# ramosian-glider/syzkaller

Hardware: AMD Instinct MI355X
Metric: coverage PCs triaged/sec vs corpus signal (+ % HBM roofline), 1/2/4/8 MI355X (higher is better)
Workload: dtype u32

## Files before the change

### syzkaller_amd/csrc/sg_bucket.hip

```cpp
#include "sg_part.h"

namespace sg {

#ifndef SG_BTHREADS
#define SG_BTHREADS 512
#endif
constexpr int kBThreads = SG_BTHREADS;
constexpr int kBWaves = kBThreads == 512 ? 6 : 8;
constexpr int kBU = 4;
constexpr uint32_t kHash = 8192;
constexpr uint32_t kMaxProbe = 31;
constexpr uint32_t kEmpty = 0xFFFFFFFFu;

struct BucketArgs {
  const uint32_t* in;
  const uint4* bdesc;
  const uint32_t* gbnd;
  uint32_t NG;
  uint32_t* mwords;
  const uint32_t* owords;
  uint32_t* nwords;
  uint8_t* rec_new;
  uint32_t* spill;
  uint32_t* nspill;
  uint32_t* ticket;
  const uint32_t* blist_b;
  const uint4* blist_q;
  const uint32_t* nlist;
  uint32_t win, win_shift;
  const uint32_t* fsum;
  uint64_t* dbg;
  uint2* pairs;
  unsigned long long* npairs;
  uint32_t rec_base;
  uint32_t nshards;
  unsigned long long* shard_cnt;
  uint32_t update;
  unsigned long long* gcur;
  const uint64_t* goff;
};

__device__ __forceinline__ uint32_t shard_of(uint32_t s, uint32_t nshards) {
  s ^= s >> 16;
  s *= 0x85EBCA6Bu;
  s ^= s >> 13;
  s *= 0xC2B2AE35u;
  s ^= s >> 16;
  return (uint32_t)(((uint64_t)s * nshards) >> 32);
}

constexpr uint32_t kMaxShards = 64;

template <int kPer>
__device__ __forceinline__ void emit_pairs(const BucketArgs& a, const uint32_t (&sig)[kPer], const uint32_t (&rec)[kPer],
                                           uint32_t* shcnt) {
  constexpr uint32_t kNone = 0xFFFFFFFFu;
  __shared__ uint32_t ewc[16];
  __shared__ unsigned long long ebase;
  const int lane = threadIdx.x & 63, w = threadIdx.x >> 6, nw = blockDim.x >> 6;
  uint32_t c = 0;
#pragma unroll
  for (int k = 0; k < kPer; k++) c += rec[k] != kNone ? 1u : 0u;
  uint32_t incl = c;
#pragma unroll
  for (int o = 1; o < 64; o <<= 1) {
    const uint32_t y = __shfl_up(incl, o);
    if (lane >= o) incl += y;
  }
  if (lane == 63) ewc[w] = incl;
  __syncthreads();
  if (threadIdx.x == 0) {
    uint32_t acc = 0;
    for (int i = 0; i < nw; i++) {
      const uint32_t v = ewc[i];
      ewc[i] = acc;
      acc += v;
    }
    ebase = acc ? atomicAdd(a.npairs, (unsigned long long)acc) : 0ull;
  }
  __syncthreads();
  uint64_t pos = ebase + ewc[w] + incl - c;
#pragma unroll
  for (int k = 0; k < kPer; k++)
    if (rec[k] != kNone) {
      a.pairs[pos++] = make_uint2(sig[k], a.rec_base + rec[k]);
      if (a.shard_cnt) atomicAdd(&shcnt[shard_of(sig[k], a.nshards)], 1u);
    }
  __syncthreads();
}

template <int kPer>
__device__ __forceinline__ void emit_grouped(const BucketArgs& a, const uint32_t (&sig)[kPer], const uint32_t (&rec)[kPer],
                                             uint32_t* lcnt, unsigned long long* lbase) {
  constexpr uint32_t kNone = 0xFFFFFFFFu;
#pragma unroll
  for (int k = 0; k < kPer; k++)
    if (rec[k] != kNone) atomicAdd(&lcnt[rec[k] >> kGroupBits], 1u);
  __syncthreads();
  for (uint32_t g = threadIdx.x; g < a.NG; g += blockDim.x) {
    const uint32_t c = lcnt[g];
    lbase[g] = c ? a.goff[(uint64_t)g << kGroupBits] + atomicAdd(&a.gcur[g], (unsigned long long)c) : 0ull;
    lcnt[g] = 0;
  }
  __syncthreads();
#pragma unroll
  for (int k = 0; k < kPer; k++)
    if (rec[k] != kNone) {
      const uint32_t g = rec[k] >> kGroupBits;
      a.pairs[lbase[g] + atomicAdd(&lcnt[g], 1u)] = make_uint2(sig[k], rec[k]);
    }
  __syncthreads();
  for (uint32_t g = threadIdx.x; g < a.NG; g += blockDim.x) lcnt[g] = 0;
  __syncthreads();
// ... 57 lines not shown
  for (int j = 0; j < kWPT; j++) {
    P.msw[j] = m[j];
    P.nsw[j] = nw[j];
  }
  const uint32_t* gr = a.gbnd + (uint64_t)b * a.NG;
#pragma unroll
  for (int j = 0; j < (int)kGroupWords; j++) {
    const uint32_t i = j * kBThreads + threadIdx.x;
    P.gw[j] = i < a.NG ? gr[i] : 0u;
  }
}

__device__ __forceinline__ uint32_t list_bucket(const BucketArgs& a, uint32_t t, uint32_t l0, uint32_t nl, uint4* q) {
  if (t >= nl) return kNumBuckets;
  *q = a.blist_q[l0 + t];
  return a.blist_b[l0 + t];
}

__device__ __forceinline__ bool fs_full(const uint32_t* fs, uint32_t rec) {
  return (fs[rec >> (kFsBits + 5)] >> ((rec >> kFsBits) & 31u)) & 1u;
}

__global__ __launch_bounds__(256) void k_flag_summary(const uint8_t* __restrict__ rec_new, uint32_t nrec,
                                                      uint32_t* __restrict__ sum, uint32_t* __restrict__ nfull) {
  const uint32_t blk = blockIdx.x * 4 + (threadIdx.x >> 6), lane = threadIdx.x & 63;
  if (blk >= (nrec + kFsRecs - 1) >> kFsBits) return;
  bool full = true;
#pragma unroll
  for (int j = 0; j < 4; j++) {
    const uint32_t i = blk * kFsRecs + j * 1024 + lane * 16;
    if (i + 16 <= nrec && ((uintptr_t)(rec_new + i) & 15) == 0) {
      const uint4 v = *reinterpret_cast<const uint4*>(rec_new + i);
      for (uint32_t w : {v.x, v.y, v.z, v.w}) full &= ((w - 0x01010101u) & ~w & 0x80808080u) == 0;
    } else {
      for (uint32_t k = i; k < i + 16 && k < nrec; k++) full &= rec_new[k] != 0;
    }
  }
  if (__all(full) && lane == 0) {
    atomicOr(&sum[blk >> 5], 1u << (blk & 31));
    atomicAdd(nfull, 1u);
  }
}

__device__ __forceinline__ uint4 uni(uint4 v) { return make_uint4(uni(v.x), uni(v.y), uni(v.z), uni(v.w)); }

constexpr uint32_t kMapMul = 0x6F4Bu;
constexpr uint32_t inv16(uint32_t c) {
  uint32_t x = c;
  for (int i = 0; i < 4; i++) x = (x * (2u - c * x)) & 0xFFFFu;
  return x;
}
constexpr uint32_t kMapInv = inv16(kMapMul);
static_assert(((kMapMul * kMapInv) & 0xFFFFu) == 1u, "kMapInv");
static_assert(kHash == 8192 && kMaxProbe <= 31, "13-bit slots, 5-bit displacements");
static_assert((uint64_t)kMaxGroups << kGroupBits <= (1u << 24), "records fit 24 bits");
constexpr uint32_t kRecMask = 0xFFFFFFu;

__device__ __forceinline__ uint32_t map_signal(uint32_t slot, uint32_t v) {
  const uint32_t home = (slot - ((v >> 24) & 31u)) & (kHash - 1);
  return (((home << 3) | (v >> 29)) * kMapInv) & 0xFFFFu;
}

__device__ __forceinline__ bool map_insert(uint32_t* ht, uint32_t sl, uint32_t rec, uint32_t disp0 = 0) {
  const uint32_t y = (sl * kMapMul) & 0xFFFFu;
  const uint32_t home = y >> 3, tag = y & 7u;
  for (uint32_t disp = disp0; disp < kMaxProbe; disp++) {
    const uint32_t mine = (tag << 29) | (disp << 24) | rec;
    uint32_t* slot = &ht[(home + disp) & (kHash - 1)];
    const uint32_t old = atomicCAS(slot, kEmpty, mine);
    if (old == kEmpty) return true;
    if ((old >> 24) == (mine >> 24)) {
      if ((old & kRecMask) > rec) atomicMin(slot, mine);
      return true;
    }
  }
  return false;
}

__device__ __forceinline__ uint32_t take_ticket(uint32_t* p) { return atomicAdd(p, 1u); }

template <bool kDbg, int kEmit, bool kSkip = false>
__global__ __launch_bounds__(kBThreads) __attribute__((amdgpu_waves_per_eu(kBWaves))) void k_bucket(BucketArgs a) {
  static_assert(!kSkip || kEmit == 0, "the summary guards flag stores");
  __shared__ uint32_t fsum[kSkip ? kFsWords : 1];
  __shared__ uint32_t mslice[kBucketWords];
  __shared__ uint32_t nbits[kBucketWords];
  __shared__ uint32_t ht[kHash];
  __shared__ alignas(16) uint32_t gb[kMaxGroups];
  __shared__ uint32_t sh_fail;
  __shared__ uint32_t sh_b[2];
  __shared__ uint4 sh_q[2];
  __shared__ uint32_t shcnt[kEmit == 1 ? kMaxShards : 1];
  __shared__ uint32_t lcnt[kEmit == 2 ? kMaxGroups : 1];
  __shared__ unsigned long long lbase[kEmit == 2 ? kMaxGroups : 1];
  const int tid = threadIdx.x;
  if (kEmit == 1)
    for (uint32_t i = tid; i < kMaxShards; i += kBThreads) shcnt[i] = 0;
  if (kEmit == 2)
    for (uint32_t i = tid; i < kMaxGroups; i += kBThreads) lcnt[i] = 0;
  const uint32_t NG = a.NG;
  constexpr uint32_t kRound = kBThreads * kBU;
  const uint64_t t_start = kDbg ? wall_clock64() : 0;
  uint64_t n_buckets = 0, n_rounds = 0;
  uint64_t ph[7] = {0, 0, 0, 0, 0, 0, 0};
  uint64_t tk = kDbg ? clock64() : 0;
  for (uint32_t i = tid; i < kHash; i += kBThreads) ht[i] = kEmpty;
  for (uint32_t i = tid; i < kBucketWords; i += kBThreads) nbits[i] = 0;
  if (tid == 0) sh_fail = 0;
  if (kSkip)
    for (uint32_t i = tid; i < kFsWords; i += kBThreads) fsum[i] = a.fsum[i];
  uint32_t nl = *a.nlist, l0 = 0;
  if (a.win) {
    const uint32_t na = nl >> a.win_shift;
    l0 = a.win == 2 ? na : 0;
    nl = a.win == 2 ? nl - na : na;
  }
  uint32_t pend_t = 0;
  if (tid == 0) {
    uint4 q0 = make_uint4(0, 0, 0, 0), q1 = make_uint4(0, 0, 0, 0);
    sh_b[0] = list_bucket(a, blockIdx.x, l0, nl, &q0);
    sh_q[0] = q0;
    sh_b[1] = list_bucket(a, gridDim.x + blockIdx.x, l0, nl, &q1);
    sh_q[1] = q1;
    pend_t = take_ticket(a.ticket);
  }
  __syncthreads();
  uint32_t b = uni(sh_b[0]), b1 = uni(sh_b[1]);
  uint4 q = uni(sh_q[0]), q1 = uni(sh_q[1]);
  if (b >= kNumBuckets) {
    if (kDbg && tid == 0) {
      for (int j = 0; j < 8; j++) a.dbg[8 * blockIdx.x + j] = 0;
      a.dbg[8 * blockIdx.x] = t_start;
      a.dbg[8 * blockIdx.x + 1] = wall_clock64();
    }
    return;
  }
  uint32_t x[kBU], y[kBU];
  BucketPre P;
  bucket_round_load(a, q.x & ~3u, q.y, x);
  bucket_pre_load(a, b, P);
  while (b < kNumBuckets) {
    const uint32_t lo = q.x, hi = q.y;
    __syncthreads();
    {
      wvec mv;
#pragma unroll
      for (int j = 0; j < kWPT; j++) mv[j] = P.msw[j];
      reinterpret_cast<wvec*>(mslice)[tid] = mv;
    }
    uint32_t ns[kWPT];
#pragma unroll
    for (int j = 0; j < kWPT; j++) ns[j] = P.nsw[j];
#pragma unroll
    for (int j = 0; j < (int)kGroupWords; j++) {
      const uint32_t i = j * kBThreads + tid;
      if (i < kMaxGroups) gb[i] = i < NG ? P.gw[j] : kEmpty;
    }
    uint32_t pend_b = kNumBuckets;
    uint4 pend_q = make_uint4(0, 0, 0, 0);
    if (tid == 0) {
      pend_b = list_bucket(a, 2 * gridDim.x + pend_t, l0, nl, &pend_q);
      pend_t = take_ticket(a.ticket);
      sh_fail = 0;
    }
    __syncthreads();
    const uint32_t gbl = NG <= 64 ? gb[threadIdx.x & 63] : kEmpty;
// ... 217 lines not shown
        for (int j = 0; j < kWPT; j++)
          if (nb[j]) {
            a.mwords[w0 + j] = mw[j] | nb[j];
            if (a.nwords) a.nwords[w0 + j] = ns[j] | nb[j];
          }
      } else if (a.nwords) {
        const wvec nb = reinterpret_cast<const wvec*>(nbits)[tid];
        uint32_t* ng = a.nwords + bucket_word(b, kWPT * tid);
#pragma unroll
        for (int j = 0; j < kWPT; j++)
          if (nb[j]) ng[j] = ns[j] | nb[j];
      }
      reinterpret_cast<wvec*>(nbits)[tid] = wvec{};
    } else {
      constexpr int kOwn = kHash / kBThreads;
      {
#pragma unroll
        for (int k = 0; k < kOwn; k++) {
          const uint32_t i = k * kBThreads + tid;
          const uint32_t v = ht[i];
          ht[i] = kEmpty;
          if (v != kEmpty) {
            const uint32_t sl = map_signal(i, v);
            atomicOr(&nbits[sl >> 5], 1u << (sl & 31));
            if (!kSkip || !fs_full(fsum, v & kRecMask)) a.rec_new[v & kRecMask] = 1;
          }
        }
        __syncthreads();
      }
      {
        const uint64_t w0 = bucket_word(b, kWPT * tid);
        uint32_t* mg = a.mwords + w0;
        uint32_t* ng = a.nwords ? a.nwords + w0 : nullptr;
        const wvec nb = reinterpret_cast<const wvec*>(nbits)[tid];
        uint32_t any = 0;
#pragma unroll
        for (int j = 0; j < kWPT; j++) any |= nb[j];
        if (any) {
          const wvec mw = reinterpret_cast<const wvec*>(mslice)[tid];
#pragma unroll
          for (int j = 0; j < kWPT; j++)
            if (nb[j]) {
              mg[j] = mw[j] | nb[j];
              if (ng) ng[j] = ns[j] | nb[j];
            }
          reinterpret_cast<wvec*>(nbits)[tid] = wvec{};
        }
      }
    }
    if (kDbg) {
      const uint64_t t = clock64();
      ph[3] += t - tk;
      tk = t;
    }
    __syncthreads();
    if (kDbg) {
      const uint64_t t = clock64();
      ph[6] += t - tk;
      tk = t;
    }
    b = b1;
    q = q1;
    b1 = uni(sh_b[0]);
    q1 = uni(sh_q[0]);
#pragma unroll
    for (int u = 0; u < kBU; u++) x[u] = y[u];
  }
  if (kEmit == 1) {
    __syncthreads();
    flush_shard_counts(a, shcnt);
  }
  if (kDbg && tid == 0) {
    a.dbg[8 * blockIdx.x] = t_start;
    a.dbg[8 * blockIdx.x + 1] = wall_clock64();
    a.dbg[8 * blockIdx.x + 2] = n_buckets;
    a.dbg[8 * blockIdx.x + 3] = n_rounds;
    for (int j = 0; j < 4; j++) a.dbg[8 * blockIdx.x + 4 + j] = ph[j];
    a.dbg[8 * gridDim.x + 3 * blockIdx.x] = ph[4];
    a.dbg[8 * gridDim.x + 3 * blockIdx.x + 1] = ph[5];
    a.dbg[8 * gridDim.x + 3 * blockIdx.x + 2] = ph[6];
  }
}

constexpr int kDThreads = 1024;
template <bool kEmit>
__global__ __launch_bounds__(kDThreads) void k_bucket_direct(BucketArgs a) {
  constexpr uint32_t kQ = 8192, kNQ = 65536 / kQ, kQW = kQ / 32;
  __shared__ uint32_t owner[kQ];
  __shared__ uint32_t mpart[kQW];
  __shared__ uint32_t nbits[kQW];
  __shared__ uint32_t gb[kMaxGroups];
  __shared__ uint32_t shcnt[kEmit ? kMaxShards : 1];
  __shared__ uint32_t lcnt[kEmit ? kMaxGroups : 1];
  __shared__ unsigned long long lbase[kEmit ? kMaxGroups : 1];
  __shared__ uint32_t fsum[kEmit ? 1 : kFsWords];
  const int tid = threadIdx.x;
  const uint32_t nsp = *a.nspill, NG = a.NG;
  if (!kEmit)
    for (uint32_t i = tid; i < kFsWords; i += kDThreads) fsum[i] = a.fsum ? a.fsum[i] : 0u;
  if (kEmit) {
    for (uint32_t i = tid; i < kMaxShards; i += kDThreads) shcnt[i] = 0;
    for (uint32_t i = tid; i < kMaxGroups; i += kDThreads) lcnt[i] = 0;
    __syncthreads();
  }
  for (uint32_t job = blockIdx.x; job < nsp * kNQ; job += gridDim.x) {
    const uint32_t b = a.spill[job / kNQ], qq = job % kNQ;
    const uint4 q = a.bdesc[b];
    for (uint32_t i = tid; i < kQW; i += kDThreads) {
      const uint64_t w = bucket_word(b, qq * kQW + i);
      mpart[i] = a.mwords[w] | (a.owords ? a.owords[w] : 0u);
      nbits[i] = 0;
    }
    for (uint32_t i = tid; i < NG; i += kDThreads) gb[i] = a.gbnd[(uint64_t)b * NG + i];
    for (uint32_t i = tid; i < kQ; i += kDThreads) owner[i] = kEmpty;
    __syncthreads();
    for (uint32_t i = q.x + tid; i < q.y; i += kDThreads) {
      const uint32_t x = a.in[i];
      const uint32_t sl = x >> 16, sq = sl % kQ;
      if (sl / kQ != qq || ((mpart[sq >> 5] >> (sq & 31)) & 1u)) continue;
      atomicMin(&owner[sq], entry_record(group_of(gb, NG, i), x));
      atomicOr(&nbits[sq >> 5], 1u << (sq & 31));
    }
    __syncthreads();
    if (kEmit) {
      constexpr int kPer = kQ / kDThreads;
      uint32_t sig[kPer], rec[kPer];
#pragma unroll
      for (int k = 0; k < kPer; k++) {
        const uint32_t i = k * kDThreads + tid;
        sig[k] = part_sig((b << 16) | (qq * kQ + i));
        rec[k] = owner[i];
      }
      if (a.gcur)
        emit_grouped(a, sig, rec, lcnt, lbase);
      else
        emit_pairs(a, sig, rec, shcnt);
      for (uint32_t i = tid; i < kQW; i += kDThreads) {
        const uint32_t nb = nbits[i];
        if (!nb) continue;
        const uint64_t w = bucket_word(b, qq * kQW + i);
        if (a.update) a.mwords[w] = mpart[i] | nb;
        if (a.nwords) a.nwords[w] |= nb;
      }
    } else {
      for (uint32_t i = tid; i < kQ; i += kDThreads)
        if (owner[i] != kEmpty && !fs_full(fsum, owner[i])) a.rec_new[owner[i]] = 1;
      for (uint32_t i = tid; i < kQW; i += kDThreads) {
        const uint32_t nb = nbits[i];
        if (nb) {
          const uint64_t w = bucket_word(b, qq * kQW + i);
          a.mwords[w] = mpart[i] | nb;
          if (a.nwords) a.nwords[w] |= nb;
        }
      }
    }
    __syncthreads();
  }
  if (kEmit) flush_shard_counts(a, shcnt);
}

uint32_t persistent_grid(sg_ctx* ctx, const void* kernel, int threads) {
  static std::mutex mu;
  static std::map<std::pair<int, const void*>, uint32_t> cache;
  std::lock_guard<std::mutex> lock(mu);
  const auto key = std::make_pair(ctx->device, kernel);
  auto it = cache.find(key);
// ... 4 lines not shown
  if (hipDeviceGetAttribute(&cus, hipDeviceAttributeMultiprocessorCount, ctx->device) != hipSuccess || cus < 1)
    cus = 256;
  const uint32_t grid = (uint32_t)(per_cu * cus);
  cache[key] = grid;
  return grid;
}

constexpr double kFsQueued = 0.9997;
static bool fs_split(sg_ctx* ctx) {
  const int64_t o = ctx->opt[kOptFlagSkip];
  if (o >= 0) return o != 0;
  m0f_poll(ctx);
  return ctx->m0f_queued >= kFsQueued;
}

int buckets_one(sg_ctx* ctx, const BucketPlan& bp, uint32_t* mwords, uint32_t* nwords, uint8_t* d_rec_new,
                const EmitArgs* emit, const uint32_t* owords) {
  const uint64_t nrec = bp.nrec;
  const uint32_t* gcount = bp.at<uint32_t>(ctx, kCB) + bp.ng;
  uint4* bdesc = bp.at<uint4>(ctx, kBD);
  uint32_t* nspill = bp.at<uint32_t>(ctx, kSP);
  const bool dbg = ctx->debug_part;
  BucketArgs ba{};
  ba.in = bp.at<uint32_t>(ctx, kV2);
  ba.bdesc = bdesc;
  ba.gbnd = bp.at<uint32_t>(ctx, kGB);
  ba.NG = (uint32_t)bp.NG;
  ba.mwords = mwords;
  ba.owords = owords;
  ba.nwords = nwords;
  ba.rec_new = d_rec_new;
  ba.nspill = nspill;
  ba.spill = nspill + 1;
  ba.ticket = bp.at<uint32_t>(ctx, kTK);
  if (emit) {
    ba.pairs = emit->pairs;
    ba.npairs = emit->npairs;
    ba.rec_base = emit->rec_base;
    ba.nshards = emit->nshards;
    ba.shard_cnt = emit->shard_cnt;
    ba.update = emit->update ? 1u : 0u;
    ba.gcur = emit->gcur;
    ba.goff = emit->goff;
  }
  uint32_t bgrid = persistent_grid(ctx, (const void*)k_bucket<false, 0>, kBThreads);
  const int64_t cap_blocks = ctx->opt[kOptBucketBlocks];
  if (cap_blocks > 0 && (uint64_t)cap_blocks < bgrid) bgrid = (uint32_t)cap_blocks;
  DevBuf<uint64_t> ddbg;
  if (dbg) {
    const int rc = ddbg.grow_drop((size_t)bgrid * 11, nullptr);
    if (rc) return rc;
    ba.dbg = ddbg.p;
  }
  const bool split = !emit && !dbg && d_rec_new && nrec <= kMaxLaunchRecords && fs_split(ctx);
  uint32_t* fsum = ba.ticket + 4;
  uint32_t* fcnt = &ctx->dev.p->fs_full_blocks;
  if (split) {
    int rc = ctx->fs_ev.create(hipEventDisableTiming);
    if (!rc) rc = m0f_host_alloc(ctx);
    if (rc) return rc;
    SG_HIP(hipMemsetAsync(fcnt, 0, 4, ctx->stream));
  }
  SG_HIP(hipMemsetAsync(ba.ticket, 0, split ? 16 + kFsWords * 4 : 4, ctx->stream));
  SG_HIP(hipMemsetAsync(nspill, 0, 4, ctx->stream));
  ba.blist_b = bp.at<uint32_t>(ctx, kLB);
  ba.blist_q = bp.at<uint4>(ctx, kLQ);
  ba.nlist = bp.at<uint32_t>(ctx, kBP) + kNumBuckets;
  {
    ScopedTimer tm(ctx, "bucket_triage");
    if (split) {
      ba.win = 1;
      ba.win_shift = (uint32_t)ctx->opt[kOptFlagSkipSplit];
    }
    auto kb = emit  ? (emit->gcur ? k_bucket<false, 2> : k_bucket<false, 1>)
              : dbg ? k_bucket<true, 0>
                    : k_bucket<false, 0>;
    hipLaunchKernelGGL(kb, dim3(bgrid), dim3(kBThreads), 0, ctx->stream, ba);
    if (split) {
      hipLaunchKernelGGL(k_flag_summary, dim3(div_up(div_up(nrec, kFsRecs), 4)), dim3(256), 0, ctx->stream,
                         (const uint8_t*)d_rec_new, (uint32_t)nrec, fsum, fcnt);
      ba.win = 2;
      ba.ticket++;
      ba.fsum = fsum;
      hipLaunchKernelGGL((k_bucket<false, 0, true>), dim3(bgrid), dim3(kBThreads), 0, ctx->stream, ba);
    }
  }
  if (split) {
    SG_HIP(hipMemcpyAsync(&ctx->pinned.p->fs_full_blocks, fcnt, 4, hipMemcpyDeviceToHost, ctx->stream));
    SG_HIP(hipEventRecord(ctx->fs_ev, ctx->stream));
    ctx->fs_pending = true;
    ctx->fs_used++;
  }
  {
    ScopedTimer tm(ctx, "bucket_spill");
    auto kd = emit ? k_bucket_direct<true> : k_bucket_direct<false>;
    hipLaunchKernelGGL(kd, dim3(512), dim3(kDThreads), 0, ctx->stream, ba);
  }
  SG_HIP(hipGetLastError());
  if (dbg) {
    uint32_t g = 0, sp = 0;
    SG_HIP(hipMemcpyAsync(&g, gcount, 4, hipMemcpyDeviceToHost, ctx->stream));
    SG_HIP(hipMemcpyAsync(&sp, nspill, 4, hipMemcpyDeviceToHost, ctx->stream));
    SG_HIP(hipStreamSynchronize(ctx->stream));
    fprintf(stderr, "sg part: n=%llu nrec=%llu tiles=%llu chunks=%u (bound %llu) spilled_buckets=%u\n",
            (unsigned long long)bp.n, (unsigned long long)nrec, (unsigned long long)bp.T, g,
            (unsigned long long)bp.gmax, sp);
    std::vector<uint4> bd(kNumBuckets);
    std::vector<uint64_t> hd((size_t)bgrid * 11);
    SG_HIP(hipMemcpy(bd.data(), bdesc, bd.size() * 16, hipMemcpyDeviceToHost));
    SG_HIP(hipMemcpy(hd.data(), ddbg.p, hd.size() * 8, hipMemcpyDeviceToHost));
    double qa = 0, qb = 0, qc = 0;
    for (uint32_t i = 0; i < bgrid; i++) {
      qa += hd[8 * bgrid + 3 * i];
      qb += hd[8 * bgrid + 3 * i + 1];
      qc += hd[8 * bgrid + 3 * i + 2];
    }
    std::vector<uint32_t> sz(kNumBuckets);
    uint64_t rounds = 0;
    for (uint32_t b = 0; b < kNumBuckets; b++) {
      sz[b] = bd[b].y - bd[b].x;
      rounds += (sz[b] + 8191) / 8192;
    }
    std::sort(sz.begin(), sz.end());
    uint64_t t0 = ~0ull, t1 = 0;
    std::vector<double> dur;
    uint64_t maxr = 0;
    double phs[4] = {0, 0, 0, 0}, nbk = 0, nrd = 0;
    for (uint32_t i = 0; i < bgrid; i++) {
      t0 = std::min(t0, hd[8 * i]);
      t1 = std::max(t1, hd[8 * i + 1]);
      dur.push_back((hd[8 * i + 1] - hd[8 * i]) / 100.0);
      maxr = std::max(maxr, hd[8 * i + 3]);
      nbk += hd[8 * i + 2];
      nrd += hd[8 * i + 3];
      for (int j = 0; j < 4; j++) phs[j] += hd[8 * i + 4 + j];
    }
    fprintf(stderr, "sg bucket per bucket (cycles, wave 0): install %.0f | rounds: test %.0f insert %.0f tail %.0f | "
            "end barrier %.0f flush %.0f final barrier %.0f | rounds/bucket %.2f\n", phs[0] / nbk, qa / nbk, qb / nbk,
            phs[1] / nbk, phs[2] / nbk, phs[3] / nbk, qc / nbk, nrd / nbk);
    std::sort(dur.begin(), dur.end());
    fprintf(stderr,
            "sg bucket: sizes max=%u p99=%u median=%u rounds=%llu | blocks=%u span=%.1fus dur min=%.1f med=%.1f "
            "max=%.1f us, max rounds/block=%llu\n",
            sz.back(), sz[kNumBuckets * 99 / 100], sz[kNumBuckets / 2], (unsigned long long)rounds, bgrid,
            (t1 - t0) / 100.0, dur.front(), dur[dur.size() / 2], dur.back(), (unsigned long long)maxr);
  }
  return SG_OK;
}

}
```

### syzkaller_amd/csrc/sg_ctx.hip

```cpp
#include "sg_internal.h"

#include <cstring>
#include <memory>

namespace sg {

static thread_local std::string g_err;

void set_error(const char* fmt, ...) {
  char buf[512];
  va_list ap;
  va_start(ap, fmt);
  vsnprintf(buf, sizeof(buf), fmt, ap);
  va_end(ap);
  g_err = buf;
}

int hip_fail(hipError_t e, const char* what) {
  set_error("HIP error %d (%s) in %s", (int)e, hipGetErrorString(e), what);
  if (e == hipErrorOutOfMemory) return SG_ENOMEM;
  if (e == hipErrorNoDevice || e == hipErrorInvalidDevice || e == hipErrorNoBinaryForGpu) return SG_ENODEV;
  return SG_EHIP;
}

// ... 241 lines not shown
  if (!ctx || tag == 0xFFFFFFFFu) return SG_EINVAL;
  std::lock_guard<std::mutex> g(ctx->mu);
  int rc = ensure_device(ctx);
  if (rc) return rc;
  if (end)
    hipLaunchKernelGGL(k_mark_end, dim3(1), dim3(1), 0, ctx->stream, (uint32_t*)&ctx->dev.p->scalar, tag);
  else
    hipLaunchKernelGGL(k_mark_begin, dim3(1), dim3(1), 0, ctx->stream, (uint32_t*)&ctx->dev.p->scalar, tag);
  SG_HIP(hipGetLastError());
  return SG_OK;
}

int sg_ctx_set_option(sg_ctx* ctx, const char* key, int64_t value) {
  if (!ctx || !key) return SG_EINVAL;
  std::lock_guard<std::mutex> g(ctx->mu);
  if (!strcmp(key, "max_launch_records")) {
    if (value < 0 || (uint64_t)value > kMaxLaunchRecords) {
      set_error("sg_ctx_set_option: max_launch_records in 1..%llu (0: the default)",
                (unsigned long long)kMaxLaunchRecords);
      return SG_EINVAL;
    }
    ctx->max_launch_recs = value ? (uint64_t)value : kMaxLaunchRecords;
    return SG_OK;
  }
  if (!strcmp(key, "owner_key_space")) {
    if (ctx->owner.p) {
      set_error("sg_ctx_set_option: owner_key_space is set before the first-owner table exists");
      return SG_EINVAL;
    }
    if (value < 0 || (uint64_t)value > 0xFFFFFFFFull) {
      set_error("sg_ctx_set_option: owner_key_space in 1..2^32-1 (0: the default)");
      return SG_EINVAL;
    }
    ctx->owner_key_space = value ? (uint64_t)value : 0xFFFFFFFFull;
    return SG_OK;
  }
  if (!strcmp(key, "debug_part")) {
    ctx->debug_part = value != 0;
    return SG_OK;
  }
  for (int i = 0; i < kOptCount; i++) {
    const SgOptRow& o = kSgOpts[i];
    if (strcmp(key, o.name)) continue;
    if (value < o.lo || value > o.hi) {
      set_error("sg_ctx_set_option: %s in %lld..%lld", key, (long long)o.lo, (long long)o.hi);
      return SG_EINVAL;
    }
    ctx->opt[i] = value;
    return SG_OK;
  }
  set_error("sg_ctx_set_option: unknown option '%s'", key);
  return SG_EINVAL;
}

int sg_ctx_get_option(sg_ctx* ctx, const char* key, int64_t* out) {
  if (!ctx || !key || !out) return SG_EINVAL;
  std::lock_guard<std::mutex> g(ctx->mu);
  if (!strcmp(key, "max_launch_records")) {
    *out = (int64_t)ctx->max_launch_recs;
    return SG_OK;
  }
  if (!strcmp(key, "owner_key_space")) {
    *out = (int64_t)ctx->owner_key_space;
    return SG_OK;
  }
  if (!strcmp(key, "debug_part")) {
    *out = ctx->debug_part;
    return SG_OK;
  }
  for (int i = 0; i < kOptCount; i++)
    if (!strcmp(key, kSgOpts[i].name)) {
      *out = ctx->opt[i];
      return SG_OK;
    }
  set_error("sg_ctx_get_option: unknown option '%s'", key);
  return SG_EINVAL;
}

}

namespace {
typedef uint64_t Quad[4];
enum CtrKind { kHost, kHost4, kDev32, kDev64, kConst, kCalc };
enum CtrCalc : uint64_t { kOwnerFloor, kM0Queued, kM0Logh, kCpuQuota, kFsFullBlocks, kWsBytes };
#define SG_DEV(field) offsetof(CtxDev, field)
struct Counter {
  const char* name;
  CtrKind kind;
  uint64_t arg;
  uint64_t sg_ctx::*host = nullptr;
  Quad sg_ctx::*host4 = nullptr;
};
const Counter kCounters[] = {
    {"owner_resets", kHost, 0, &sg_ctx::owner_resets},
    {"owner_floor", kCalc, kOwnerFloor},
    {"owner_key_space", kHost, 0, &sg_ctx::owner_key_space},
    {"max_launch_records", kHost, 0, &sg_ctx::max_launch_recs},
    {"host_copy_bytes", kHost, 0, &sg_ctx::host_copy_bytes},
    {"host_copy_ns", kHost, 0, &sg_ctx::host_copy_ns},
    {"host_wait_ns", kHost, 0, &sg_ctx::host_wait_ns},
    {"host_copy_threads", kHost, 0, &sg_ctx::host_threads},
    {"m0_filter_used", kHost, 0, &sg_ctx::m0f_used},
    {"m0_filter_fallback", kHost, 0, &sg_ctx::m0f_fallback},
    {"m0_filter_survivors", kHost, 0, &sg_ctx::m0f_survivors},
    {"m0_filter_queued_milli", kCalc, kM0Queued},
    {"m0_filter_halves_log", kCalc, kM0Logh},
    {"flag_skip_used", kHost, 0, &sg_ctx::fs_used},
    {"flag_skip_full_blocks", kCalc, kFsFullBlocks},
    {"hints_candidates", kHost, 0, &sg_ctx::hints_cands},
    {"exec_comps_general", kHost, 0, &sg_ctx::exec_comps_general},
    {"exec_cover_general", kHost, 0, &sg_ctx::exec_cover_general},
    {"merge_pairs_generic", kHost4, 0, nullptr, &sg_ctx::merge_pairs},
    {"merge_pairs_diff_small", kHost4, 1, nullptr, &sg_ctx::merge_pairs},
    {"merge_pairs_gap", kHost4, 2, nullptr, &sg_ctx::merge_pairs},
    {"merge_pairs_tile", kHost4, 3, nullptr, &sg_ctx::merge_pairs},
    {"canon_wave_lists", kHost4, 0, nullptr, &sg_ctx::canon_stats},
    {"canon_block_lists", kHost4, 1, nullptr, &sg_ctx::canon_stats},
    {"canon_big_segments", kHost4, 2, nullptr, &sg_ctx::canon_stats},
    {"canon_merge_passes", kHost4, 3, nullptr, &sg_ctx::canon_stats},
    {"owned_big_records", kDev32, SG_DEV(owned_big)},
    {"triage_runs_wide", kDev32, SG_DEV(tr_wide)},
    {"triage_runs_copied", kDev32, SG_DEV(tr_route[kTrCopied])},
    {"triage_runs_sorted", kDev32, SG_DEV(tr_route[kTrSorted])},
    {"triage_runs_ranked", kDev32, SG_DEV(tr_route[kTrRanked])},
    {"triage_runs_foreach", kDev32, SG_DEV(tr_route[kTrForeach])},
    {"prio_bad_ids", kDev64, SG_DEV(prio_bad_ids)},
    {"sha1_long_progs", kDev64, SG_DEV(sha1_long_progs)},
    {"sha1_long_len", kConst, kSha1Long},
    {"inflate_long_streams", kDev64, SG_DEV(inflate_long_streams)},
    {"inflate_long_len", kConst, kInflateLong},
    {"prio_band_cells", kConst, kPrioBandCells},
    {"prio_short_len", kConst, kPrioShort},
    {"triage_runs_sort_cap", kConst, kTrSort},
    {"tinput_chunk", kConst, kTinChunk},
    {"exec_comps_fast_cap", kConst, SG_EXEC_COMPS_FAST_CAP},
    {"exec_cover_fast_cap", kConst, SG_EXEC_COVER_FAST_CAP},
    {"cpu_quota_milli", kCalc, kCpuQuota},
    {"workspace_bytes", kCalc, kWsBytes},
};

int counter_calc(sg_ctx* ctx, uint64_t which, uint64_t* out) {
  if (which == kFsFullBlocks && ctx->fs_pending) {
    SG_HIP(hipEventSynchronize(ctx->fs_ev));
    ctx->fs_pending = false;
    ctx->fs_full_blocks = ctx->pinned.p->fs_full_blocks;
  }
  switch (which) {
    case kOwnerFloor: *out = ctx->owner.p ? ctx->owner_floor : ctx->owner_key_space; break;
    case kM0Queued: *out = ctx->m0f_queued < 0 ? ~0ull : (uint64_t)(ctx->m0f_queued * 1000.0 + 0.5); break;
    case kM0Logh: *out = (uint64_t)ctx->m0f_logh; break;
    case kCpuQuota: *out = (uint64_t)(ctx->cpu_quota * 1000.0 + 0.5); break;
    case kFsFullBlocks: *out = ctx->fs_full_blocks; break;
    case kWsBytes: *out = ctx->ws.cap; break;
  }
  return SG_OK;
}
}

extern "C" int sg_ctx_counter(sg_ctx* ctx, const char* name, uint64_t* out) {
  if (!ctx || !name || !out) return SG_EINVAL;
  std::lock_guard<std::mutex> g(ctx->mu);
  for (const Counter& c : kCounters) {
    if (strcmp(name, c.name)) continue;
    if (c.kind == kCalc) return counter_calc(ctx, c.arg, out);
    uint64_t v = c.kind == kConst ? c.arg : 0;
    if (c.kind == kHost) v = ctx->*c.host;
    if (c.kind == kHost4) v = (ctx->*c.host4)[c.arg];
    if (c.kind == kDev32 || c.kind == kDev64) {
      SG_HIP(hipStreamSynchronize(ctx->stream));
      SG_HIP(hipMemcpy(&v, (const char*)ctx->dev.p + c.arg, c.kind == kDev64 ? 8 : 4, hipMemcpyDeviceToHost));
    }
    *out = v;
    return SG_OK;
  }
  set_error("sg_ctx_counter: unknown counter '%s'", name);
  return SG_EINVAL;
}
```

### syzkaller_amd/csrc/sg_internal.h

```cpp
#pragma once

#include <hip/hip_runtime.h>

#include <cstdarg>
#include <cstddef>
#include <cstdint>
#include <cstdio>
#include <deque>
#include <map>
#include <mutex>
#include <string>
#include <vector>

#include "../../include/syzsig.h"
#include "sg_buf.h"
#include "sg_opts.h"
#include "sg_plan.h"

namespace sg {

constexpr uint64_t kSetWords = 1ull << 27;
constexpr uint64_t kSetBytes = kSetWords * 4;
constexpr uint64_t kOwnerEntries = 1ull << 32;
constexpr uint32_t kOwnerInf = 0xFFFFFFFFu;
constexpr uint64_t kMaxLaunchRecords = 1ull << 24;

constexpr int kBlock = 256;
constexpr int kChunk = 256;
constexpr int kTile = 4096;
constexpr int kChunksPerTile = kTile / kChunk;
constexpr int kWin = 1024;

void set_error(const char* fmt, ...);

struct KernelTimer {
  bool enabled = false;
  struct Rec {
    int id;
    hipEvent_t a, b;
  };
  std::vector<Rec> pending;
  std::vector<hipEvent_t> pool;
  std::deque<Event> events;
  std::map<std::string, int> ids;
  std::vector<std::string> names;
  std::vector<double> ms;
  std::vector<uint64_t> count;
};

}

struct PrefixSlice {
  uint64_t r0, r1, e0, e1;
  size_t ws_base;
};

struct PrefixSlot {
  std::vector<PrefixSlice> slices;
  uint64_t nrec = 0;
  uint64_t n = 0;
  uint32_t* marks = nullptr;
  bool keep = false;
  bool open = false;
  sg::DevBuf<char> ws;
};
constexpr uint32_t kPrefixSlots = 2;

namespace sg {
enum : uint32_t { kTrCopied = 0, kTrSorted = 1, kTrRanked = 2, kTrForeach = 3, kTrRoutes = 4 };
struct CtxDev {
  uint64_t scalar;
  uint32_t m0f_queued;
  uint32_t fs_full_blocks;
  uint32_t owned_big;
  uint32_t tr_wide;
  uint32_t tr_route[kTrRoutes];
  uint64_t prio_bad_ids, sha1_long_progs, inflate_long_streams;
};
static_assert(offsetof(CtxDev, scalar) % 8 == 0 && offsetof(CtxDev, prio_bad_ids) % 8 == 0 &&
                  offsetof(CtxDev, sha1_long_progs) % 8 == 0 && offsetof(CtxDev, inflate_long_streams) % 8 == 0,
              "64-bit device words are 8-byte aligned");
static_assert(offsetof(CtxDev, tr_route) == offsetof(CtxDev, tr_wide) + 4, "wide and the routes are zeroed together");
struct CtxPinned {
  uint32_t m0f_queued;
  uint32_t fs_full_blocks;
};
}

struct sg_ctx {
  int device = 0;
  sg::Stream own_stream;
  hipStream_t stream = nullptr;
  sg::Stream copy_stream;
  sg::Event pipe_ev[4];
  int64_t opt[kOptCount];
  sg_ctx() { for (int i = 0; i < kOptCount; i++) opt[i] = kSgOpts[i].def; }
  sg::DevBuf<sg::CtxDev> dev;
  sg::DevBuf<char> m0f;
  sg::Buf<sg::CtxPinned, true> pinned;
  sg::Event m0f_ev;
  int m0f_last = -1;
  bool m0f_pending = false;
  uint64_t m0f_nrec = 0;
  double m0f_queued = -1;
  uint64_t m0f_used = 0, m0f_fallback = 0, m0f_survivors = 0;
  uint32_t m0f_backoff = 0, m0f_skip = 0;
  uint64_t fs_used = 0, fs_full_blocks = 0;
  sg::Event fs_ev;
  bool fs_pending = false;
  int m0f_logh = 0;
  double cpu_quota = 0;
  uint64_t host_copy_bytes = 0, host_copy_ns = 0, host_wait_ns = 0, host_threads = 0;
  uint64_t hints_cands = 0;
  uint64_t exec_comps_general = 0;
  uint64_t exec_cover_general = 0;
  uint64_t merge_pairs[4] = {0, 0, 0, 0};
  uint64_t canon_stats[4] = {0, 0, 0, 0};
  sg::DevBuf<char> ws;
  sg::PinBuf pin;
  sg::DevBuf<char> dstage;
  sg::DevBuf<uint8_t> inflate_out;
  sg::DevBuf<uint32_t> owner;
  uint64_t owner_floor = 0;
  uint64_t owner_key_space = 0xFFFFFFFFull;
  uint64_t owner_resets = 0;
  uint64_t max_launch_recs = 0;
  PrefixSlot prefix[kPrefixSlots];
  bool debug_part = false;
  sg::DevBuf<uint64_t> slice_off;
  sg::DevBuf<uint64_t> slice_cuts;
  sg::DevBuf<uint32_t> gen_prob, gen_alias, gen_perm;
  uint64_t gen_seed = 0;
  double gen_s = 0;
  uint32_t gen_nranks = 0;
  sg::KernelTimer timer;
  std::mutex mu;
};

struct sg_set {
  sg_ctx* ctx = nullptr;
  uint32_t* words = nullptr;
  sg::DevBuf<uint32_t> mem;
};

struct SigKey {
  uint32_t w[SG_SIG_BYTES / 4];
};
struct SigHalf {
  sg::DevBuf<SigKey> store;
  sg::DevBuf<uint32_t> table;
  uint32_t* keys() const { return (uint32_t*)store.p; }
  uint32_t mask() const { return (uint32_t)(table.cap - 1); }
  void swap(SigHalf& o) {
    store.swap(o.store);
    table.swap(o.table);
  }
};
struct sg_sigset {
  sg_ctx* ctx = nullptr;
  uint64_t count = 0;
  SigHalf cur;
  SigHalf next;
};

namespace sg {

int ensure_device(sg_ctx* ctx);
int ws_reserve(sg_ctx* ctx, size_t bytes);
int ws_reserve(sg_ctx* ctx, const WsPlan& plan);
inline void* ws_at(sg_ctx* ctx, size_t off) { return ctx->ws.p + off; }
int pin_reserve(sg_ctx* ctx, size_t bytes);
int dstage_reserve(sg_ctx* ctx, size_t bytes);
int dstage_reserve(sg_ctx* ctx, const WsPlan& plan);
template <typename T>
inline T* dstage_at(sg_ctx* ctx, size_t off) {
  return (T*)(ctx->dstage.p + off);
}
constexpr size_t kRecFloor = 1024;
template <typename T>
int rec_reserve(sg_ctx* ctx, DevBuf<T>& b, size_t need, size_t keep) {
  return b.grow_keep(grow_cap(b.cap, need, kRecFloor), keep, ctx->stream);
}
int slice_off_reserve(sg_ctx* ctx, size_t n);
int upload(sg_ctx* ctx, void* d_dst, const void* h_src, size_t bytes);
int csr_download(sg_ctx* ctx, uint64_t* h_off, const uint64_t* d_off, uint64_t n, void* h_vals, const void* d_vals,
                 size_t elem, uint64_t cap);
int owner_keys(sg_ctx* ctx, uint64_t nkeys, uint32_t* key_lo);

void timer_begin(sg_ctx* ctx, const char* name, int* slot);
void timer_end(sg_ctx* ctx, int slot);
// ... 219 lines not shown
```

Measured before the change: 133.7 billion.

## Add set-only bucket kernel for second window when every record is already flagged

When the flag summary shows that every summary block is fully flagged, the second-window k_bucket pass now exits at once. A new lightweight persistent kernel, k_bucket_sets, runs instead. It only ORs the new coverage bits into the mask and new-word arrays, with no hash table, record-ownership tracking or flag stores. Its loads of the next bucket and its mask words are double-buffered. The goal is to avoid the heavy per-record dedup machinery when no record can change state, at the cost of one extra launch and a device-side check in both kernels. A new counter reports how often this path was taken.

```diff
diff --git a/syzkaller_amd/csrc/sg_bucket.hip b/syzkaller_amd/csrc/sg_bucket.hip
--- a/syzkaller_amd/csrc/sg_bucket.hip
+++ b/syzkaller_amd/csrc/sg_bucket.hip
@@ -29,6 +29,9 @@
   const uint32_t* nlist;
   uint32_t win, win_shift;
   const uint32_t* fsum;
+  const uint32_t* fs_cnt;
+  uint32_t fs_nblk;
+  uint32_t* fs_all;
   uint64_t* dbg;
   uint2* pairs;
   unsigned long long* npairs;
@@ -252,6 +255,7 @@
 template <bool kDbg, int kEmit, bool kSkip = false>
 __global__ __launch_bounds__(kBThreads) __attribute__((amdgpu_waves_per_eu(kBWaves))) void k_bucket(BucketArgs a) {
   static_assert(!kSkip || kEmit == 0, "the summary guards flag stores");
+  if (kSkip && *a.fs_cnt == a.fs_nblk) return;
   __shared__ uint32_t fsum[kSkip ? kFsWords : 1];
   __shared__ uint32_t mslice[kBucketWords];
   __shared__ uint32_t nbits[kBucketWords];
@@ -635,6 +639,148 @@
   }
 }
 
+constexpr int kSQ = 2;
+constexpr uint32_t kSQuad = kBThreads * 4;
+constexpr uint32_t kSRound = kSQuad * kSQ;
+struct SetsPre {
+  uint32_t msw[kWPT];
+  uint32_t nsw[kWPT];
+};
+
+__device__ __forceinline__ uint32_t sets_pos(uint32_t base, int j) { return base + j * kSQuad + threadIdx.x * 4; }
+
+__device__ __forceinline__ void sets_round_load(const BucketArgs& a, uint32_t base, uint32_t hi, v4u32 (&x)[kSQ]) {
+#pragma unroll
+  for (int j = 0; j < kSQ; j++) {
+    x[j] = v4u32{0, 0, 0, 0};
+    const uint32_t p = sets_pos(base, j);
+    if (p < hi) x[j] = __builtin_nontemporal_load(reinterpret_cast<const v4u32*>(a.in + p));
+  }
+}
+
+__device__ __forceinline__ void sets_pre_load(const BucketArgs& a, uint32_t b, SetsPre& P) {
+  const uint64_t w0 = bucket_word(b, kWPT * threadIdx.x);
+  wvec m = *reinterpret_cast<const wvec*>(a.mwords + w0);
+  if (a.owords) m |= *reinterpret_cast<const wvec*>(a.owords + w0);
+  wvec nw = {};
+  if (a.nwords) nw = *reinterpret_cast<const wvec*>(a.nwords + w0);
+#pragma unroll
+  for (int j = 0; j < kWPT; j++) {
+    P.msw[j] = m[j];
+    P.nsw[j] = nw[j];
+  }
+}
+
+__global__ __launch_bounds__(kBThreads) __attribute__((amdgpu_waves_per_eu(8))) void k_bucket_sets(BucketArgs a) {
+  if (*a.fs_cnt != a.fs_nblk) return;
+  __shared__ alignas(16) uint32_t mslice[kBucketWords];
+  __shared__ alignas(16) uint32_t nbits[kBucketWords];
+  __shared__ uint32_t sh_b[2];
+  __shared__ uint4 sh_q[2];
+  const int tid = threadIdx.x;
+  uint32_t nl = *a.nlist, l0 = 0;
+  if (a.win) {
+    const uint32_t na = nl >> a.win_shift;
+    l0 = a.win == 2 ? na : 0;
+    nl = a.win == 2 ? nl - na : na;
+  }
+  uint32_t pend_t = 0;
+  if (tid == 0) {
+    uint4 q0 = make_uint4(0, 0, 0, 0), q1 = make_uint4(0, 0, 0, 0);
+    sh_b[0] = list_bucket(a, blockIdx.x, l0, nl, &q0);
+    sh_q[0] = q0;
+    sh_b[1] = list_bucket(a, gridDim.x + blockIdx.x, l0, nl, &q1);
+    sh_q[1] = q1;
+    pend_t = take_ticket(a.ticket);
+    if (blockIdx.x == 0) atomicAdd(a.fs_all, 1u);
+  }
+  __syncthreads();
+  uint32_t b = uni(sh_b[0]), b1 = uni(sh_b[1]);
+  uint4 q = uni(sh_q[0]), q1 = uni(sh_q[1]);
+  if (b >= kNumBuckets) return;
+  v4u32 x[kSQ], y[kSQ];
+  SetsPre P;
+  sets_round_load(a, q.x & ~3u, q.y, x);
+  sets_pre_load(a, b, P);
+  wvec ns;
+  {
+    wvec mv;
+#pragma unroll
+    for (int j = 0; j < kWPT; j++) {
+      mv[j] = P.msw[j];
+      ns[j] = P.nsw[j];
+    }
+    reinterpret_cast<wvec*>(mslice)[tid] = mv;
+    reinterpret_cast<wvec*>(nbits)[tid] = wvec{};
+  }
+  __syncthreads();
+  while (b < kNumBuckets) {
+    const uint32_t lo = q.x, hi = q.y;
+    uint32_t pend_b = kNumBuckets;
+    uint4 pend_q = make_uint4(0, 0, 0, 0);
+    if (tid == 0) {
+      pend_b = list_bucket(a, 2 * gridDim.x + pend_t, l0, nl, &pend_q);
+      pend_t = take_ticket(a.ticket);
+    }
+    for (uint32_t base = lo & ~3u;;) {
+      const uint32_t next = base + kSRound;
+      const bool last = next >= hi;
+      if (!last || b1 < kNumBuckets) sets_round_load(a, last ? q1.x & ~3u : next, last ? q1.y : hi, y);
+      if (last && b1 < kNumBuckets) sets_pre_load(a, b1, P);
+#pragma unroll
+      for (int j = 0; j < kSQ; j++) {
+        uint32_t mw[4];
+#pragma unroll
+        for (int u = 0; u < 4; u++) mw[u] = mslice[x[j][u] >> 21];
+#pragma unroll
+        for (int u = 0; u < 4; u++) {
+          const uint32_t i = sets_pos(base, j) + u, v = x[j][u];
+          const uint32_t bit = 1u << ((v >> 16) & 31);
+          if (i >= lo && i < hi && !(mw[u] & bit)) atomicOr(&nbits[v >> 21], bit);
+        }
+      }
+#pragma unroll
+      for (int j = 0; j < kSQ; j++) x[j] = y[j];
+      if (last) break;
+      base = next;
+    }
+    if (tid == 0) {
+      sh_b[0] = pend_b;
+      sh_q[0] = pend_q;
+    }
+    __syncthreads();
+    {
+      const uint64_t w0 = bucket_word(b, kWPT * tid);
+      const wvec nb = reinterpret_cast<const wvec*>(nbits)[tid];
+      const wvec cm = reinterpret_cast<const wvec*>(mslice)[tid];
+      uint32_t any = 0;
+#pragma unroll
+      for (int j = 0; j < kWPT; j++) {
+        any |= nb[j];
+        if (nb[j]) {
+          a.mwords[w0 + j] = cm[j] | nb[j];
+          if (a.nwords) a.nwords[w0 + j] = ns[j] | nb[j];
+        }
+      }
+      if (any) reinterpret_cast<wvec*>(nbits)[tid] = wvec{};
+      if (b1 < kNumBuckets) {
+        wvec mv;
+#pragma unroll
+        for (int j = 0; j < kWPT; j++) {
+          mv[j] = P.msw[j];
+          ns[j] = P.nsw[j];
+        }
+        reinterpret_cast<wvec*>(mslice)[tid] = mv;
+      }
+    }
+    b = b1;
+    q = q1;
+    b1 = uni(sh_b[0]);
+    q1 = uni(sh_q[0]);
+    __syncthreads();
+  }
+}
+
 constexpr int kDThreads = 1024;
 template <bool kEmit>
 __global__ __launch_bounds__(kDThreads) void k_bucket_direct(BucketArgs a) {
@@ -805,11 +951,22 @@
       ba.win = 2;
       ba.ticket++;
       ba.fsum = fsum;
+      ba.fs_cnt = fcnt;
+      ba.fs_nblk = (uint32_t)div_up(nrec, kFsRecs);
+      ba.fs_all = &ctx->dev.p->fs_all_flagged;
       hipLaunchKernelGGL((k_bucket<false, 0, true>), dim3(bgrid), dim3(kBThreads), 0, ctx->stream, ba);
+      BucketArgs bs = ba;
+      bs.ticket = ba.ticket + 1;
+      uint32_t sgrid = persistent_grid(ctx, (const void*)k_bucket_sets, kBThreads);
+      if (cap_blocks > 0 && (uint64_t)cap_blocks < sgrid) sgrid = (uint32_t)cap_blocks;
+      hipLaunchKernelGGL(k_bucket_sets, dim3(sgrid), dim3(kBThreads), 0, ctx->stream, bs);
     }
   }
   if (split) {
-    SG_HIP(hipMemcpyAsync(&ctx->pinned.p->fs_full_blocks, fcnt, 4, hipMemcpyDeviceToHost, ctx->stream));
+    static_assert(offsetof(CtxDev, fs_all_flagged) == offsetof(CtxDev, fs_full_blocks) + 4 &&
+                      offsetof(CtxPinned, fs_all_flagged) == offsetof(CtxPinned, fs_full_blocks) + 4,
+                  "the two words travel in one copy");
+    SG_HIP(hipMemcpyAsync(&ctx->pinned.p->fs_full_blocks, fcnt, 8, hipMemcpyDeviceToHost, ctx->stream));
     SG_HIP(hipEventRecord(ctx->fs_ev, ctx->stream));
     ctx->fs_pending = true;
     ctx->fs_used++;
diff --git a/syzkaller_amd/csrc/sg_ctx.hip b/syzkaller_amd/csrc/sg_ctx.hip
--- a/syzkaller_amd/csrc/sg_ctx.hip
+++ b/syzkaller_amd/csrc/sg_ctx.hip
@@ -347,7 +347,7 @@
 namespace {
 typedef uint64_t Quad[4];
 enum CtrKind { kHost, kHost4, kDev32, kDev64, kConst, kCalc };
-enum CtrCalc : uint64_t { kOwnerFloor, kM0Queued, kM0Logh, kCpuQuota, kFsFullBlocks, kWsBytes };
+enum CtrCalc : uint64_t { kOwnerFloor, kM0Queued, kM0Logh, kCpuQuota, kFsFullBlocks, kFsAllFlagged, kWsBytes };
 #define SG_DEV(field) offsetof(CtxDev, field)
 struct Counter {
   const char* name;
@@ -372,6 +372,7 @@
     {"m0_filter_halves_log", kCalc, kM0Logh},
     {"flag_skip_used", kHost, 0, &sg_ctx::fs_used},
     {"flag_skip_full_blocks", kCalc, kFsFullBlocks},
+    {"flag_skip_all_flagged", kCalc, kFsAllFlagged},
     {"hints_candidates", kHost, 0, &sg_ctx::hints_cands},
     {"exec_comps_general", kHost, 0, &sg_ctx::exec_comps_general},
     {"exec_cover_general", kHost, 0, &sg_ctx::exec_cover_general},
@@ -405,10 +406,11 @@
 };
 
 int counter_calc(sg_ctx* ctx, uint64_t which, uint64_t* out) {
-  if (which == kFsFullBlocks && ctx->fs_pending) {
+  if ((which == kFsFullBlocks || which == kFsAllFlagged) && ctx->fs_pending) {
     SG_HIP(hipEventSynchronize(ctx->fs_ev));
     ctx->fs_pending = false;
     ctx->fs_full_blocks = ctx->pinned.p->fs_full_blocks;
+    ctx->fs_all_flagged = ctx->pinned.p->fs_all_flagged;
   }
   switch (which) {
     case kOwnerFloor: *out = ctx->owner.p ? ctx->owner_floor : ctx->owner_key_space; break;
@@ -416,6 +418,7 @@
     case kM0Logh: *out = (uint64_t)ctx->m0f_logh; break;
     case kCpuQuota: *out = (uint64_t)(ctx->cpu_quota * 1000.0 + 0.5); break;
     case kFsFullBlocks: *out = ctx->fs_full_blocks; break;
+    case kFsAllFlagged: *out = ctx->fs_all_flagged; break;
     case kWsBytes: *out = ctx->ws.cap; break;
   }
   return SG_OK;
diff --git a/syzkaller_amd/csrc/sg_internal.h b/syzkaller_amd/csrc/sg_internal.h
--- a/syzkaller_amd/csrc/sg_internal.h
+++ b/syzkaller_amd/csrc/sg_internal.h
@@ -72,6 +72,7 @@
   uint64_t scalar;
   uint32_t m0f_queued;
   uint32_t fs_full_blocks;
+  uint32_t fs_all_flagged;
   uint32_t owned_big;
   uint32_t tr_wide;
   uint32_t tr_route[kTrRoutes];
@@ -84,6 +85,7 @@
 struct CtxPinned {
   uint32_t m0f_queued;
   uint32_t fs_full_blocks;
+  uint32_t fs_all_flagged;
 };
 }
 
@@ -105,7 +107,7 @@
   double m0f_queued = -1;
   uint64_t m0f_used = 0, m0f_fallback = 0, m0f_survivors = 0;
   uint32_t m0f_backoff = 0, m0f_skip = 0;
-  uint64_t fs_used = 0, fs_full_blocks = 0;
+  uint64_t fs_used = 0, fs_full_blocks = 0, fs_all_flagged = 0;
   sg::Event fs_ev;
   bool fs_pending = false;
   int m0f_logh = 0;
```

Result: faster. 154.2 billion, median of 6 (+15.3%).
